# sanweiliti/EgoHMR

Hardware: AMD Instinct MI355X
Metric: sampled bodies/sec (100-step DDPM, batch 256) (higher is better)
Workload: dtype f32 results: denoiser GEMMs as 3x f16 MFMA on hi/lo-split operands (f32 accumulate) on the last 100 of 100 steps, plain f16 operands on the first 0; k = 100 is~; 1 GPU; B256 S1 DDPM-100 N4096 ResNet50+PointNet cond, diffuse_fuse(2 GCN passes), LBS every step, unguided; items_per_gpu=256, samples_per_item=1, denoising_steps=100, scene_points=4096, lbs_every_step=True, collision_guided=False, gcn_precision=f16x3, f16x3_last_steps=100, parallelism=items sharded x1, one RCCL all-gather of [B,226] at the end

## Files before the change

### egohmr_amd/csrc/gcn.hip

```cpp
#include <stdlib.h>

#include "common.h"
#include "egohmr_hip.h"
#include "gcn_dev.h"
#include "internal.h"

namespace {

__global__ void pack_w_kernel(const float* __restrict__ W, float* __restrict__ Wp, int K, int N) {
  __shared__ float tile[32][33];
  int u = blockIdx.z;
  int k0 = blockIdx.y * 32, n0 = blockIdx.x * 32;
  int tx = threadIdx.x & 31, ty = threadIdx.x >> 5;
  for (int r = ty; r < 32; r += 8) {
    int k = k0 + r, n = n0 + tx;
    tile[r][tx] = (k < K && n < N) ? W[((size_t)u * K + k) * N + n] : 0.f;
  }
  __syncthreads();
  for (int r = ty; r < 32; r += 8) {
    int n = n0 + r, k = k0 + tx;
    if (n < N && k < K) {
      int nt = n >> 6, c = n & 63;
      Wp[((size_t)nt * 128 + u * 64 + c) * K + k] = tile[tx][r];
    }
// ... 139 lines not shown
#pragma unroll
      for (int u = 0; u < 2; ++u) b[u] = *(const f32x4*)(Bs + (rB + 64 * u) * BK + cB);
#pragma unroll
      for (int s = 0; s < 4; ++s) {
#pragma unroll
        for (int t = 0; t < 3; ++t) {
          acc0[t] = __builtin_amdgcn_mfma_f32_32x32x2f32(a[t][s], b[0][s], acc0[t], 0, 0, 0);
          acc1[t] = __builtin_amdgcn_mfma_f32_32x32x2f32(a[t][s], b[1][s], acc1[t], 0, 0, 0);
        }
      }
    }
  }

  const int n = n_tile * BNH + 32 * wn + mi;
  const size_t rowb = m0 + 96 * wm + 48 * h;
  float res0[kJ], res1[kJ];
#pragma unroll
  for (int j = 0; j < kJ; ++j) res0[j] = RES ? Res[(rowb + j) * (size_t)N + n] : 0.f;
  {
    float dj[kJ], mj[kJ];
    const float sh = L.shift[n];
#pragma unroll
    for (int j = 0; j < kJ; ++j) { dj[j] = L.D[j * N + n]; mj[j] = L.M1[j * N + n]; }
    __builtin_amdgcn_sched_barrier(0);
#pragma unroll
    for (int j = 0; j < kJ; ++j) {
#pragma unroll
      for (int beta = 0; beta < 2; ++beta) {
        const int q = 24 * beta + j;
        acc0[q >> 4][q & 15] = fmaf(dj[j], acc0[q >> 4][q & 15], sh);
        acc1[q >> 4][q & 15] *= mj[j];
      }
    }
  }
  __builtin_amdgcn_sched_barrier(0);
#pragma unroll
  for (int j = 0; j < kJ; ++j) res1[j] = RES ? Res[(rowb + 24 + j) * (size_t)N + n] : 0.f;
  __builtin_amdgcn_sched_barrier(0);
  {
    float d0[kJ], g1[kJ];
#pragma unroll
    for (int j = 0; j < kJ; ++j) { d0[j] = acc0[j >> 4][j & 15]; g1[j] = acc1[j >> 4][j & 15]; }
    gcn_mix_store<false>(d0, g1, res0, n, N, rowb, L.Aoff, Y, L.relu != 0);
  }
  __builtin_amdgcn_sched_barrier(0);
  {
    float d0[kJ], g1[kJ];
#pragma unroll
    for (int j = 0; j < kJ; ++j) { d0[j] = acc0[(24 + j) >> 4][(24 + j) & 15]; g1[j] = acc1[(24 + j) >> 4][(24 + j) & 15]; }
    gcn_mix_store<false>(d0, g1, res1, n, N, rowb + 24, L.Aoff, Y, L.relu != 0);
  }
}

template <int OUT>
__global__ __launch_bounds__(256) void gcn_input_kernel(GcnInputArgs a) {
  __shared__ __attribute__((aligned(16))) float T[kJ * 256];
  gcn_input_body<OUT>(T, blockIdx.x, blockIdx.y, a);
}

template <int OUT>
__global__ __launch_bounds__(256) void gcn_input_rows_kernel(GcnInputArgs a) {
  __shared__ __attribute__((aligned(16))) float T[kJ * 256];
  gcn_input_body<OUT, false, true>(T, (int)threadIdx.x, blockIdx.x, blockIdx.y, a, nullptr);
}


template <bool HALF_IN>
__global__ __launch_bounds__(256) void gcn_out_dot_kernel(const float* __restrict__ X, OutDev O, float* __restrict__ hs, int64_t rows) {
  __shared__ float part[4][16][16];
  gcn_out_dot_rows16<HALF_IN, 0>(X, O, hs, (int64_t)blockIdx.x * OUT_ROWS_PER_BLOCK, rows, part, (int)threadIdx.x);
}

__global__ __launch_bounds__(192) void gcn_out_mix_kernel(const float* __restrict__ hs, OutDev O, const uint8_t* __restrict__ vis,
                                                          float* __restrict__ x0, int B, int passes, const int32_t* __restrict__ mask_slot) {
  __shared__ float sh[2][kJ][12];
  __shared__ float outs[2][kJ][6];
  const int b = blockIdx.x, tid = threadIdx.x;
  const int slot = mask_slot ? mask_slot[b] : b;
  for (int i = tid; i < passes * kJ * 12; i += 192) {
    const int p = i / (kJ * 12), rem = i % (kJ * 12);
    sh[p][rem / 12][rem % 12] = (p == 1 && slot < 0) ? 0.f : hs[((size_t)(p ? B + slot : b) * kJ) * 12 + rem];
  }
  __syncthreads();
  for (int e = tid; e < passes * kJ * 6; e += 192) {
    const int p = e / (kJ * 6), j = (e / 6) % kJ, c = e % 6;
    const float s = O.A[j * kJ + j] * (O.M[j * 6 + c] * sh[p][j][c]);
    float t = 0.f;
    for (int jp = 0; jp < kJ; ++jp)
      if (jp != j) t = fmaf(O.A[j * kJ + jp], O.M[jp * 6 + c] * sh[p][jp][6 + c], t);
    outs[p][j][c] = s + t + O.bias[c];
  }
  __syncthreads();
  if (tid < kPoseDim) {
    const int j = tid / 6, c = tid % 6;
    float v = outs[0][j][c];
    if (passes == 2 && !vis[(size_t)b * kJ + j]) v = outs[1][j][c];
    x0[(size_t)b * kPoseDim + tid] = v;
  }
}

}

__global__ void pack_aoff_half_kernel(const float* __restrict__ Aoff, half8* __restrict__ out) {
  const int lane = threadIdx.x, i = lane & 31;
#pragma unroll
  for (int s = 0; s < 3; ++s) {
    half8 v;
#pragma unroll
    for (int c = 0; c < 8; ++c) {
      const int kk = 16 * s + 8 * (lane >> 5) + c;
// ... 102 lines not shown
    hipLaunchKernelGGL(pack_out_kernel, dim3((unsigned)ceil_div(12 * hid_dim, 256)), dim3(256), 0, st, adj, *output_conv,
                       g->out.Wt, g->out.M, g->out.A, g->out.bias);
    if (hipGetLastError() != hipSuccess) rc = EHM_EIO;
  }
  if (rc == 0 && num_hidden > 0) {
    if (hipMalloc(&g->hidden_dev, sizeof(LayerDev) * num_hidden) != hipSuccess ||
        hipMemcpyAsync(g->hidden_dev, g->hidden, sizeof(LayerDev) * num_hidden, hipMemcpyHostToDevice, st) != hipSuccess)
      rc = EHM_ENOMEM;
  }
  if (rc == 0 && (hipMalloc(&g->chain_sticky, 64) != hipSuccess || hipMemsetAsync(g->chain_sticky, 0, 64, st) != hipSuccess)) rc = EHM_ENOMEM;
  if (rc == 0 && hipStreamSynchronize(st) != hipSuccess) rc = EHM_EIO;
  if (rc == 0) rc = ehm_gcn_reserve_rows(g, 2 * 256 * kJ);
  if (rc != 0) {
    if (g->hidden_dev) (void)hipFree(g->hidden_dev);
    if (g->chain_sticky) (void)hipFree(g->chain_sticky);
    if (g->chain_sync) (void)hipFree(g->chain_sync);
    if (g->hs) (void)hipFree(g->hs);
    (void)hipFree(g->arena);
    delete g;
    ehm_set_error("ehm_gcn_create: packing kernels failed");
    return rc;
  }
  *out = g;
  return 0;
}

extern "C" void ehm_gcn_destroy(ehm_gcn* h) {
  if (!h) return;
  (void)hipFree(h->arena);
  if (h->hs) (void)hipFree(h->hs);
  if (h->hidden_dev) (void)hipFree(h->hidden_dev);
  if (h->chain_sync) (void)hipFree(h->chain_sync);
  if (h->chain_sticky) (void)hipFree(h->chain_sticky);
  delete h;
}

int ehm_gcn_input_args(const ehm_gcn* h, const GcnRun& r, const float* h_img, const float* h_oth, const uint8_t* vis, const float* x, const float* Wx,
                       const float* tvec, float* out, int B, int passes, GcnInputArgs* a) {
  EHM_CHECK_ARG(h && h_img && h_oth && vis && x && Wx && tvec && out && a);
  EHM_CHECK_ARG(B > 0 && (passes == 1 || passes == 2));
  a->h_img = h_img; a->h_oth = h_oth; a->vis = vis; a->x = x; a->Wx = Wx; a->tvec = tvec;
  a->L = h->input;
  a->Y = out;
  a->B = B; a->passes = passes; a->mask_all = r.uncond_masks_all;
  a->mask_items = r.items(passes);
  a->sticky = h->chain_sticky;
  a->total_vb = r.virtual_bodies(B, passes);
  a->ny = (int)ceil_div(h->hid, 256);
  return 0;
}

template <bool PRE, int OUT>
static void launch_input_conv(const GcnInputArgs& a, hipStream_t st) {
  const dim3 grid((unsigned)a.total_vb, (unsigned)a.ny);
  if constexpr (PRE) hipLaunchKernelGGL(gcn_input_rows_kernel<OUT>, grid, dim3(256), 0, st, a);
  else hipLaunchKernelGGL(gcn_input_kernel<OUT>, grid, dim3(256), 0, st, a);
}
template <bool PRE>
static int input_conv(const GcnInputArgs& a, int fmt, hipStream_t st) {
  if (fmt == EHM_PREC_F32) launch_input_conv<PRE, 0>(a, st);
  else if (fmt == EHM_PREC_F16X3) launch_input_conv<PRE, 1>(a, st);
  else launch_input_conv<PRE, 2>(a, st);
  EHM_LAUNCH_CHECK();
  return 0;
}

int ehm_gcn_input_impl(const ehm_gcn* h, const GcnRun& r, const float* h_img, const float* h_oth, const uint8_t* vis, const float* x,
                       const float* Wx, const float* tvec, float* out, int B, int passes, hipStream_t st) {
  GcnInputArgs a;
  const int rc = ehm_gcn_input_args(h, r, h_img, h_oth, vis, x, Wx, tvec, out, B, passes, &a);
  return rc != 0 ? rc : input_conv<false>(a, gcn_input_format(h, r.precision), st);
}

extern "C" int ehm_gcn_input_layer(ehm_gcn* h, const float* h_img, const float* h_oth, const uint8_t* vis, const float* x,
                                   const float* Wx, const float* tvec, float* out, int B, int passes, void* stream) {
  EHM_CHECK_ARG(h);
  const int rc = ehm_gcn_input_impl(h, h->run, h_img, h_oth, vis, x, Wx, tvec, out, B, passes, (hipStream_t)stream);
  if (rc == 0) h->run.valid_rows = (int64_t)h->run.virtual_bodies(B, passes) * kJ;
  return rc;
}

extern "C" int ehm_gcn_input_layer_rows(ehm_gcn* h, const float* pre, float* out, int bodies, void* stream) {
  EHM_CHECK_ARG(h && pre && out && bodies > 0);
  GcnInputArgs a{};
  a.L = h->input;
  a.Y = out;
  a.B = bodies; a.passes = 1; a.mask_all = 0;
  a.mask_items = nullptr;
  a.total_vb = bodies;
  a.ny = (int)ceil_div(h->hid, 256);
  a.sticky = h->chain_sticky;
  h->run.valid_rows = (int64_t)bodies * kJ;
  a.pre = pre;
  return input_conv<true>(a, gcn_input_format(h, h->run.precision), (hipStream_t)stream);
}

static int hidden_layer(const ehm_gcn* h, const GcnRun& r, int layer, const float* X, const float* residual, float* out, int64_t rows_pad,
                        hipStream_t st) {
  EHM_CHECK_ARG(X && out);
  EHM_CHECK_ARG(layer >= 0 && layer < h->num_hidden);
  EHM_CHECK_ARG(rows_pad > 0 && rows_pad % BM == 0);
  EHM_CHECK_ARG(X != out);
  if (r.precision != EHM_PREC_F32)
    return ehm_gcn_tile_layer_impl(h, r, layer, X, residual, out, rows_pad, layer == h->num_hidden - 1, st);
  const int m_tiles = (int)(rows_pad / BM);
  const int blocks = m_tiles * (h->hid / BNH);
  if (residual)
    hipLaunchKernelGGL(gcn_hidden_kernel<true>, dim3(blocks), dim3(256), 0, st, X, h->hidden[layer], residual, out, m_tiles);
  else
    hipLaunchKernelGGL(gcn_hidden_kernel<false>, dim3(blocks), dim3(256), 0, st, X, h->hidden[layer], (const float*)nullptr, out, m_tiles);
  EHM_LAUNCH_CHECK();
  return 0;
}

extern "C" int ehm_gcn_hidden_layer(ehm_gcn* h, int layer, const float* X, const float* residual, float* out,
                                    int64_t rows_pad, void* stream) {
  EHM_CHECK_ARG(h);
  return hidden_layer(h, h->run, layer, X, residual, out, rows_pad, (hipStream_t)stream);
// ... 136 lines not shown
```

### egohmr_amd/csrc/gcn_dev.h

```cpp
#pragma once
#include "common.h"
#include "egohmr_hip.h"

typedef _Float16 half_t;
typedef _Float16 half8 __attribute__((ext_vector_type(8)));

constexpr int BM = 192;
constexpr int BNH = 64;
constexpr int BK = 32;
constexpr int A_TILE = BM * BK;
constexpr int B_TILE = 2 * BNH * BK;
constexpr int STAGE = A_TILE + B_TILE;

struct LayerDev {
  float* Wp;
  half_t* Ws;
  half_t* Wh;
  float* Ds;
  float* M1s;
  float w_scale;
  float* D;
  float* M1;
  float* shift;
  float* Aoff;
// ... 118 lines not shown
static __device__ __forceinline__ void gcn_mix_store(const float (&d0)[kJ], const float (&g1)[kJ], const float (&res)[kJ], int n, int N,
                                              size_t row0, const float* __restrict__ Aoff, float* __restrict__ Y, bool relu) {
  typedef const float __attribute__((address_space(4))) cfloat;
  const cfloat* Ac = (const cfloat*)(uintptr_t)Aoff;
#pragma unroll
  for (int j = 0; j < kJ; ++j) {
    float s = d0[j];
#pragma unroll
    for (int jp = 0; jp < kJ; ++jp) s = fmaf(Ac[j * kJ + jp], g1[jp], s);
    if (relu) s = fmaxf(s, 0.f);
    if (SPLIT_OUT) split_store_pair<G>((half_t*)Y, row0 + j, n, N, s + res[j]);
    else Y[(row0 + j) * (size_t)N + n] = s + res[j];
  }
}

typedef float f32x2 __attribute__((ext_vector_type(2)));
template <class Store>
static __device__ __forceinline__ void gcn_mix2(const f32x2 (&dp)[kJ], const f32x2 (&gp)[kJ], const float* __restrict__ Aoff, bool relu,
                                                Store store) {
  typedef const float __attribute__((address_space(4))) cfloat;
  const cfloat* Ac = (const cfloat*)(uintptr_t)Aoff;
#pragma unroll
  for (int j0 = 0; j0 < kJ; j0 += 4) {
    __builtin_amdgcn_sched_barrier(0);
#pragma unroll
    for (int i = 0; i < 4; ++i) {
      const int j = j0 + i;
      float s0 = dp[j][0], s1 = dp[j][1];
#pragma unroll
      for (int jp = 0; jp < kJ; ++jp) {
        const float a = Ac[j * kJ + jp];
        s0 = fmaf(a, gp[jp][0], s0);
        s1 = fmaf(a, gp[jp][1], s1);
      }
      if (relu) { s0 = fmaxf(s0, 0.f); s1 = fmaxf(s1, 0.f); }
      store(j, s0, s1);
    }
  }
}

constexpr unsigned int kStickySaturated = 4u;

struct GcnInputArgs {
  const float* h_img; const float* h_oth; const uint8_t* vis; const float* x; const float* Wx; const float* tvec;
  LayerDev L;
  float* Y;
  int B, passes, mask_all;
  const int32_t* mask_items;
  int total_vb, ny;
  unsigned int* sticky = nullptr;
  const float* pre = nullptr;
};

template <int OUT, bool X_LDS = false, bool PRE = false>
__device__ __forceinline__ void gcn_input_body(float* T, int tid, int bx, int by, const GcnInputArgs& a, const float* xb_in) {
  const float* __restrict__ h_img = a.h_img; const float* __restrict__ h_oth = a.h_oth; const uint8_t* __restrict__ vis = a.vis;
  const float* __restrict__ x = a.x; const float* __restrict__ Wx = a.Wx; const float* __restrict__ tvec = a.tvec;
  const LayerDev& L = a.L;
  float* __restrict__ Y = a.Y;
  const int B = a.B, passes = a.passes, mask_all = a.mask_all;
  const int32_t* __restrict__ mask_items = a.mask_items;
  (void)passes;
  const int N = L.N;
  const int vb = bx;
  const int p = vb >= B ? 1 : 0, b = p ? (mask_items ? mask_items[vb - B] : vb - B) : vb;
  const int n_raw = by * 256 + tid;
  const int n = n_raw < N ? n_raw : N - 1;
  float base[2] = {0.f, 0.f}, img[2] = {0.f, 0.f}, wx[2][6] = {{0.f, 0.f, 0.f, 0.f, 0.f, 0.f}, {0.f, 0.f, 0.f, 0.f, 0.f, 0.f}};
  if constexpr (!PRE)
#pragma unroll
  for (int k = 0; k < 2; ++k) {
    base[k] = ((p == 1 && mask_all) ? 0.f : h_oth[((size_t)b * 2 + k) * N + n]) + tvec[k * N + n];
    img[k] = (p == 0) ? h_img[((size_t)b * 2 + k) * N + n] : 0.f;
#pragma unroll
    for (int c = 0; c < 6; ++c) wx[k][c] = Wx[(k * 6 + c) * N + n];
  }
  const float* xb = xb_in ? xb_in : (PRE ? nullptr : x + (size_t)b * kPoseDim);
  float xr[X_LDS ? kPoseDim : 1];
  if constexpr (X_LDS) {
    typedef const f32x4 __attribute__((address_space(3))) lf32x4;
    lf32x4* xl = (lf32x4*)xb_in;
#pragma unroll
    for (int i = 0; i < kPoseDim / 4; ++i) {
      const f32x4 v = xl[i];
      xr[4 * i] = v[0]; xr[4 * i + 1] = v[1]; xr[4 * i + 2] = v[2]; xr[4 * i + 3] = v[3];
    }
  }
  const uint8_t* vb_ = PRE ? nullptr : vis + (size_t)b * kJ;
  float h0[kJ], h1[kJ];
  const float sh = L.shift[n];
  float dj[kJ], mj[kJ];
  {
    typedef unsigned int u32x4_tb __attribute__((ext_vector_type(4)));
    const __amdgpu_buffer_rsrc_t dsB = ehm_buffer_rsrc(L.Ds), m1B = ehm_buffer_rsrc(L.M1s);
    const unsigned int nrow = (unsigned int)n * (unsigned int)(kJ * 4);
#pragma unroll
    for (int q4 = 0; q4 < kJ / 4; ++q4) {
      const u32x4_tb d4 = __builtin_amdgcn_raw_buffer_load_b128(dsB, nrow, 16 * q4, 0);
      const u32x4_tb m4 = __builtin_amdgcn_raw_buffer_load_b128(m1B, nrow, 16 * q4, 0);
#pragma unroll
      for (int i = 0; i < 4; ++i) {
        const unsigned int du = d4[i], mu = m4[i];
        dj[4 * q4 + i] = __builtin_bit_cast(float, du);
        mj[4 * q4 + i] = __builtin_bit_cast(float, mu);
      }
    }
  }
  const f32x2 img2 = {img[0], img[1]}, base2 = {base[0], base[1]};
  f32x2 wx2[6];
#pragma unroll
  for (int c = 0; c < 6; ++c) wx2[c] = f32x2{wx[0][c], wx[1][c]};
#pragma unroll
  for (int j = 0; j < kJ; ++j) {
    f32x2 s;
    if constexpr (PRE) {
      const float* pr = a.pre + ((size_t)vb * kJ + j) * 2 * (size_t)N + n;
      s = f32x2{pr[0], pr[N]};
    } else {
    const float v = vb_[j] ? 1.f : 0.f;
    s = __builtin_elementwise_fma(f32x2{v, v}, img2, base2);
#pragma unroll
    for (int c = 0; c < 6; ++c) {
      const float xv = X_LDS ? xr[X_LDS ? j * 6 + c : 0] : xb[j * 6 + c];
      s = __builtin_elementwise_fma(f32x2{xv, xv}, wx2[c], s);
    }
    }
    h0[j] = fmaf(dj[j], s[0], sh);
    h1[j] = mj[j] * s[1];
  }
  if constexpr (OUT == 2) {
    typedef unsigned int u32x4_t __attribute__((ext_vector_type(4)));
    typedef _Float16 half2_t __attribute__((ext_vector_type(2)));
    const int lane = tid & 63, wv = tid >> 6;
    f32x16 DA, DB;
#pragma unroll
    for (int r = 0; r < 16; ++r) { DA[r] = 0.f; DB[r] = 0.f; }
#pragma unroll
    for (int s3 = 0; s3 < 3; ++s3) {
      const half8 af = ((const half8*)L.AoffH)[s3 * 64 + lane];
      u32x4_t Pw, Qw;
#pragma unroll
      for (int e = 0; e < 4; ++e) {
        const int kp = 16 * s3 + 2 * e, kq = kp + 8;
        const float p0 = kp < kJ ? h1[kp] : h0[kp - kJ], p1 = kp + 1 < kJ ? h1[kp + 1] : h0[kp + 1 - kJ];
        const float q0 = kq < kJ ? h1[kq] : h0[kq - kJ], q1 = kq + 1 < kJ ? h1[kq + 1] : h0[kq + 1 - kJ];
        const half2_t hp = {(half_t)fmaf(p0, 0.f, fminf(fmaxf(p0, -65504.f), 65504.f)), (half_t)fmaf(p1, 0.f, fminf(fmaxf(p1, -65504.f), 65504.f))};
        const half2_t hq = {(half_t)fmaf(q0, 0.f, fminf(fmaxf(q0, -65504.f), 65504.f)), (half_t)fmaf(q1, 0.f, fminf(fmaxf(q1, -65504.f), 65504.f))};
        const auto sw = __builtin_amdgcn_permlane32_swap(__builtin_bit_cast(unsigned int, hp), __builtin_bit_cast(unsigned int, hq), false, false);
        Pw[e] = sw[0];
        Qw[e] = sw[1];
      }
      DA = __builtin_amdgcn_mfma_f32_32x32x16_f16(af, __builtin_bit_cast(half8, Pw), DA, 0, 0, 0);
      DB = __builtin_amdgcn_mfma_f32_32x32x16_f16(af, __builtin_bit_cast(half8, Qw), DB, 0, 0, 0);
    }
    const bool relu = L.relu != 0;
    const int cA = 64 * wv + (lane & 31), half = lane >> 5;
#pragma unroll
    for (int r = 0; r < 12; ++r) {
      const int j = (r & 3) + 8 * (r >> 2) + 4 * half;
      const float va = relu ? fmaxf(DA[r], 0.f) : DA[r], vb = relu ? fmaxf(DB[r], 0.f) : DB[r];
      T[j * 256 + cA] = fmaf(DA[r], 0.f, va);
      T[j * 256 + cA + 32] = fmaf(DB[r], 0.f, vb);
    }
  } else {
    typedef const float __attribute__((address_space(4))) cfloat;
    const cfloat* Ac = (const cfloat*)(uintptr_t)L.Aoff;
    const bool relu = L.relu != 0;
    f32x2 sacc[kJ / 2];
#pragma unroll
    for (int jj = 0; jj < kJ / 2; ++jj) sacc[jj] = f32x2{h0[2 * jj], h0[2 * jj + 1]};
#pragma unroll
    for (int jp = 0; jp < kJ; ++jp) {
      const f32x2 hh = {h1[jp], h1[jp]};
#pragma unroll
      for (int jj = 0; jj < kJ / 2; ++jj) sacc[jj] = __builtin_elementwise_fma(f32x2{Ac[jp * kJ + 2 * jj], Ac[jp * kJ + 2 * jj + 1]}, hh, sacc[jj]);
    }
#pragma unroll
    for (int jj = 0; jj < kJ / 2; ++jj) {
      f32x2 o = sacc[jj];
      if (relu) { o[0] = fmaxf(o[0], 0.f); o[1] = fmaxf(o[1], 0.f); }
      if constexpr (OUT != 0) o = __builtin_elementwise_fma(sacc[jj], f32x2{0.f, 0.f}, o);
      T[(2 * jj) * 256 + tid] = o[0];
      T[(2 * jj + 1) * 256 + tid] = o[1];
    }
  }
  __syncthreads();
  typedef unsigned int u32x4 __attribute__((ext_vector_type(4)));
  const int nb = by * 256;
#pragma unroll
  for (int i = 0; i < 3; ++i) {
    const int u = tid + 256 * i, j = u >> 5, c8 = (u & 31) * 8;
    if (nb + c8 >= N) continue;

    const f32x4 v0 = *(const f32x4*)(T + j * 256 + c8), v1 = *(const f32x4*)(T + j * 256 + c8 + 4);
    const float v[8] = {v0[0], v0[1], v0[2], v0[3], v1[0], v1[1], v1[2], v1[3]};
    const size_t row = (size_t)vb * kJ + j;
    if (OUT != 0) {
      if (a.sticky) {
        float vm = 0.f;
#pragma unroll
        for (int k = 0; k < 8; k += 2) vm = fmaxf(vm, fmaxf(fabsf(v[k]), fabsf(v[k + 1])));
        if (vm >= 65504.f && vm <= 3.0e38f) __hip_atomic_fetch_or(a.sticky, kStickySaturated, __ATOMIC_RELAXED, __HIP_MEMORY_SCOPE_AGENT);
      }
      half8 hh, ll;
#pragma unroll
      for (int k = 0; k < 8; ++k) {
        const float c = fmaf(v[k], 0.f, fminf(fmaxf(v[k], -65504.f), 65504.f));
        hh[k] = (half_t)c;
        ll[k] = (half_t)fminf(fmaxf(v[k] - (float)hh[k], -65504.f), 65504.f);
      }
      if (OUT == 1) {
        half_t* p = (half_t*)Y + split_off<32>(row, nb + c8, N);
        *(u32x4*)p = __builtin_bit_cast(u32x4, hh);
        *(u32x4*)(p + 32) = __builtin_bit_cast(u32x4, ll);
      } else {
        *(u32x4*)((half_t*)Y + row * (size_t)N + nb + c8) = __builtin_bit_cast(u32x4, hh);
      }
    } else {
      float* p = Y + row * (size_t)N + nb + c8;
      *(f32x4*)p = v0;
      *(f32x4*)(p + 4) = v1;
    }
  }
}
template <int OUT>
__device__ __forceinline__ void gcn_input_body(float* T, int bx, int by, const GcnInputArgs& a) {
  gcn_input_body<OUT>(T, (int)threadIdx.x, bx, by, a, nullptr);
}

constexpr int OUT_ROWS_PER_BLOCK = 16;
template <bool HALF_IN, int AUX>
__device__ __forceinline__ f32x4 gcn_out_dot_quarter(const float* __restrict__ X, const OutDev& O, int64_t r, int wave, int lane) {
  const int K = O.K;
  const int row = lane & 15, q = lane >> 4;
  const int kq = K / 4;
  typedef unsigned int u32x4_od __attribute__((ext_vector_type(4)));
  typedef unsigned int u32x2_od __attribute__((ext_vector_type(2)));
  const __amdgpu_buffer_rsrc_t rsX = ehm_buffer_rsrc_4g(X), rsW = ehm_buffer_rsrc(O.Wt);
  const unsigned int vox = (unsigned int)((r * K + (size_t)wave * kq + 8 * q) * (HALF_IN ? 2 : 4));
  const unsigned int vow = (unsigned int)(((size_t)(row < 12 ? row : 0) * K + (size_t)wave * kq + 8 * q) * 4);
  f32x4 acc = {0.f, 0.f, 0.f, 0.f}, acc2 = {0.f, 0.f, 0.f, 0.f};
#pragma unroll 4
  for (int k = 0; k + 32 <= kq; k += 32) {
    float xv[8];
    if (HALF_IN) {
      const half8 hv = __builtin_bit_cast(half8, (u32x4_od)__builtin_amdgcn_raw_buffer_load_b128(rsX, vox, k * 2, AUX));
#pragma unroll
      for (int c = 0; c < 8; ++c) xv[c] = (float)hv[c];
    } else {
      const f32x4 x0 = __builtin_bit_cast(f32x4, (u32x4_od)__builtin_amdgcn_raw_buffer_load_b128(rsX, vox, k * 4, AUX));
      const f32x4 x1 = __builtin_bit_cast(f32x4, (u32x4_od)__builtin_amdgcn_raw_buffer_load_b128(rsX, vox, k * 4 + 16, AUX));
#pragma unroll
      for (int c = 0; c < 4; ++c) { xv[c] = x0[c]; xv[4 + c] = x1[c]; }
    }
    f32x4 w0 = __builtin_bit_cast(f32x4, (u32x4_od)__builtin_amdgcn_raw_buffer_load_b128(rsW, vow, k * 4, 0));
    f32x4 w1 = __builtin_bit_cast(f32x4, (u32x4_od)__builtin_amdgcn_raw_buffer_load_b128(rsW, vow, k * 4 + 16, 0));
    if (row >= 12) { w0 = f32x4{0.f, 0.f, 0.f, 0.f}; w1 = w0; }
#pragma unroll
    for (int c = 0; c < 4; c += 2) {
      acc = __builtin_amdgcn_mfma_f32_16x16x4f32(xv[c], w0[c], acc, 0, 0, 0);
      acc2 = __builtin_amdgcn_mfma_f32_16x16x4f32(xv[c + 1], w0[c + 1], acc2, 0, 0, 0);
    }
#pragma unroll
    for (int c = 0; c < 4; c += 2) {
      acc = __builtin_amdgcn_mfma_f32_16x16x4f32(xv[4 + c], w1[c], acc, 0, 0, 0);
      acc2 = __builtin_amdgcn_mfma_f32_16x16x4f32(xv[5 + c], w1[c + 1], acc2, 0, 0, 0);
    }
  }
  if (kq & 16) {
    const int k = kq - 16 - 4 * q;
    f32x4 xv;
    if (HALF_IN) {
      typedef _Float16 half4_t __attribute__((ext_vector_type(4)));
      const half4_t hv = __builtin_bit_cast(half4_t, (u32x2_od)__builtin_amdgcn_raw_buffer_load_b64(rsX, vox + (unsigned int)(k * 2), 0, AUX));
      xv = f32x4{(float)hv[0], (float)hv[1], (float)hv[2], (float)hv[3]};
    } else {
// ... 31 lines not shown
```

### egohmr_amd/csrc/internal.h

```cpp
#pragma once
#include "common.h"
#include "egohmr_hip.h"

int ehm_smpl_forward_impl(ehm_smpl* h, const float* betas, const float* rot_or_x, bool from_rot6d, const float* mean,
                          const float* std_, float* verts, float* joints, float* Rws, float* Aws, float* pose6d_out, int B,
                          hipStream_t st, float* vposed = nullptr);
int ehm_smpl_writes_vposed(const ehm_smpl* h, int B);
int ehm_smpl_pose_impl(ehm_smpl* h, const float* betas, const float* x, const float* mean, const float* std_, float* Rws, float* Aws,
                       float* jws, int B, hipStream_t st);
int ehm_step_body_impl(ehm_smpl* h, const float* hs, const void* out_dev, const uint8_t* vis, const float* x, const float* noise,
                       const float* grad, float* x_next, float* x0, const ehm_step_coefs* c, int ddim, int passes, const int32_t* mask_slot, int do_pose,
                       const float* betas, const float* mean, const float* std_, float* verts, float* joints, float* Rws, float* Aws,
                       float* pose6d, int B, hipStream_t st, const struct GcnInputArgs* next_input = nullptr, int next_prec = 0,
                       int* fused = nullptr, void* defer_pf = nullptr);
int ehm_skin_steps_impl(ehm_smpl* h, const float* A_steps, const void* pf_steps, int nsteps, int final_step, int B, float* verts, float* joints,
                        float* scratch_verts, float* scratch_joints, hipStream_t st);
int ehm_step_fused_impl(const void* out_dev, const float* X, int prec, const uint8_t* vis, const float* x, const float* noise, const float* grad,
                        float* x_next, float* x0, const ehm_step_coefs* c, int ddim, int passes, const int32_t* mask_slot, int B,
                        const struct GcnInputArgs* next_input, int next_prec, hipStream_t st);
int ehm_pose_steps_impl(ehm_smpl* smpl, const float* x0_steps, int nsteps, int final_step, int B, const float* betas, const float* mean,
                        const float* std_, float* A_steps, void* pf_steps, float* R, float* joints, float* pose6d, float* x0_final,
                        float* scratch_joints, hipStream_t st);
int ehm_skin_min_bodies();
int ehm_smpl_has_mfma_skin(const ehm_smpl* h);
int64_t ehm_skin_pf_bytes_per_step(int B);
void ehm_smpl_dev(const ehm_smpl* h, void* out);
size_t ehm_smpl_dev_size();
int ehm_smpl_num_verts(const ehm_smpl* h);
int ehm_smpl_num_extra(const ehm_smpl* h);
struct GcnInputArgs;
struct GcnRun;
int ehm_gcn_input_args(const ehm_gcn* h, const GcnRun& r, const float* h_img, const float* h_oth, const uint8_t* vis, const float* x, const float* Wx,
                       const float* tvec, float* out, int B, int passes, GcnInputArgs* a);
int ehm_gcn_input_impl(const ehm_gcn* h, const GcnRun& r, const float* h_img, const float* h_oth, const uint8_t* vis, const float* x,
                       const float* Wx, const float* tvec, float* out, int B, int passes, hipStream_t st);
int ehm_gcn_hidden_stack_impl(ehm_gcn* h, const GcnRun& r, float* const bufs[3], int64_t rows_pad, int* result_index, hipStream_t st);
int ehm_gcn_output_dot_impl(ehm_gcn* h, const GcnRun& r, const float* X, int B, int passes, const float** hs, hipStream_t st);
int ehm_num_cus();
int ehm_gcn_tile_layer_impl(const ehm_gcn* h, const GcnRun& r, int layer, const void* X, const void* residual, void* out, int64_t rows_pad,
                            bool out_f32, hipStream_t st);
int ehm_gcn_tile_chain_impl(ehm_gcn* h, const GcnRun& r, void* const bufs[3], int64_t rows_pad, hipStream_t st);
void ehm_pack_half(const float* X, void* Y, size_t n, float scale, hipStream_t st);
int ehm_gcn_reserve_rows(ehm_gcn* h, int64_t rows_pad);
int64_t ehm_guidance_scratch_bytes(int B, int N);
int ehm_guidance_impl(ehm_smpl* smpl, const float* betas, const float* x, const float* mean, const float* std_,
                      const float* scene, int B, int N, float tau, float denom, float margin, float* verts_ws, float* joints_ws, float* R_ws,
                      float* A_ws, float* gverts, float* loss, float* gpose, float* grad, void* scratch, hipStream_t st,
                      float* vposed_ws = nullptr);
unsigned long long* ehm_prof_evals_ptr();
struct EhmProfScope {
  int cls;
  hipStream_t st;
  void* rec;
  EhmProfScope(int cls_, hipStream_t st_);
  ~EhmProfScope();
};
```

### egohmr_amd/csrc/step.hip

```cpp
#include "common.h"
#include "egohmr_hip.h"
#include "gcn_dev.h"
#include "internal.h"
#include "smpl_dev.h"
#include "step_dev.h"

namespace {

struct StepFusedArgs {
  const float* X;
  StepBodyArgs sb;
  GcnInputArgs in;
  int do_input;
};

constexpr int kFusedT = kJ * 256;

template <bool HALF_IN, int OUT, int NT>
__global__ __launch_bounds__(NT, 4) void step_fused_kernel(StepFusedArgs a) {
  constexpr int G = NT / 256, NWV = NT / 64;
  __shared__ __attribute__((aligned(16))) float T[G * kFusedT];
  __shared__ __attribute__((aligned(16))) StepBodyLds L;
  const int tid = threadIdx.x, lane = tid & 63, wave = tid >> 6;
  const int b = blockIdx.x, B = a.sb.B;
  const int slot = a.sb.passes == 2 ? (a.sb.mask_slot ? a.sb.mask_slot[b] : b) : -1;
  const int nrows = slot >= 0 ? 2 * kJ : kJ;

  float (*part)[4][16][16] = (float (*)[4][16][16])T;
  for (int task = wave; task < 12; task += NWV) {
    const int tile = task >> 2, wq = task & 3;
    if (16 * tile < nrows) {
      int rr = 16 * tile + (lane & 15);
      if (rr >= nrows) rr = nrows - 1;
      const int64_t r = (int64_t)(rr >= kJ ? B + slot : b) * kJ + (rr % kJ);
      const f32x4 acc = gcn_out_dot_quarter<HALF_IN, 0>(a.X, a.sb.O, r, wq, lane);
#pragma unroll
      for (int c = 0; c < 4; ++c) part[tile][wq][4 * (lane >> 4) + c][lane & 15] = acc[c];
    }
  }
  if (wave == NWV - 1) step_stage_tables<true>(b, lane, a.sb, L);
  __syncthreads();
  for (int i = tid; i < 2 * kJ * 12; i += NT) {
    const int rr = i / 12, cc12 = i % 12, tile = rr >> 4, tr = rr & 15;
    (&L.sh[0][0][0])[i] = rr < nrows ? (part[tile][0][tr][cc12] + part[tile][1][tr][cc12]) + (part[tile][2][tr][cc12] + part[tile][3][tr][cc12]) : 0.f;
  }
  __syncthreads();
  if (wave < 3) {
    SmplDev unused;
    step_body_one<true, false, true>(b, lane, a.sb, unused, L, [] {}, wave, 3);
  }
  if (!a.do_input) return;
  __syncthreads();
  const int ny = a.in.ny, np = slot >= 0 ? 2 : 1, grp = tid >> 8;
  const int rounds = np * ((ny + G - 1) / G);
  for (int k = 0; k < rounds; ++k) {
    const int cb = grp + G * (k / np), p = k % np;
    if (cb < ny) gcn_input_body<OUT, true>(T + grp * kFusedT, tid & 255, p ? B + slot : b, cb, a.in, L.xn);
    else __syncthreads();
    __syncthreads();
  }
}

struct PoseStepsArgs {
  const float* x0_steps;
  const float *betas, *mean, *std_;
  float* A_steps; char* pf_steps; int64_t pf_bytes;
  float *R, *joints, *pose6d, *x0_final, *scratch_joints;
  int B, final_step, jstride;
};

__global__ __launch_bounds__(64) void pose_steps_kernel(PoseStepsArgs p, SmplDev S) {
  __shared__ StepBodyLds L;
  const int b = blockIdx.x, s = blockIdx.y, lane = threadIdx.x;
  const bool fin = s == p.final_step;
  StepBodyArgs a{};
  a.betas = p.betas; a.mean = p.mean; a.std_ = p.std_; a.B = p.B; a.jstride = p.jstride;
  a.Rws = fin ? p.R : nullptr;
  a.joints = fin ? p.joints : p.scratch_joints;
  a.pose6d = fin ? p.pose6d : nullptr;
  a.Aws = p.A_steps + (size_t)s * p.B * kJ * 12;
  a.pf = (sk_half8*)(p.pf_steps + (size_t)s * p.pf_bytes);
  const float* x0row = p.x0_steps + ((size_t)s * p.B + b) * kPoseDim;
  for (int e = lane; e < kPoseDim; e += 64) {
    const float v = x0row[e];
    L.x0s[e] = v;
    if (fin) p.x0_final[(size_t)b * kPoseDim + e] = v;
  }
  __syncthreads();
  step_pose_part(b, lane, a, S, L, [] { __syncthreads(); }, L.x0s);
}

template <bool HALF_IN, int NT>
void launch_fused2(int next_prec, int B, hipStream_t st, const StepFusedArgs& a) {
  const dim3 grid((unsigned)B), blk(NT);
  if (next_prec == EHM_PREC_F32) hipLaunchKernelGGL((step_fused_kernel<HALF_IN, 0, NT>), grid, blk, 0, st, a);
  else if (next_prec == EHM_PREC_F16X3) hipLaunchKernelGGL((step_fused_kernel<HALF_IN, 1, NT>), grid, blk, 0, st, a);
  else hipLaunchKernelGGL((step_fused_kernel<HALF_IN, 2, NT>), grid, blk, 0, st, a);
}
template <bool HALF_IN>
void launch_fused(int next_prec, int B, hipStream_t st, const StepFusedArgs& a) {
  if (B <= ehm_num_cus()) launch_fused2<HALF_IN, 1024>(next_prec, B, st, a);
  else if (B > 2 * ehm_num_cus()) launch_fused2<HALF_IN, 256>(next_prec, B, st, a);
  else launch_fused2<HALF_IN, 512>(next_prec, B, st, a);
}

}

int ehm_step_fused_impl(const void* out_dev, const float* X, int prec, const uint8_t* vis, const float* x, const float* noise, const float* grad,
                        float* x_next, float* x0, const ehm_step_coefs* c, int ddim, int passes, const int32_t* mask_slot, int B,
                        const GcnInputArgs* next_input, int next_prec, hipStream_t st) {
  StepFusedArgs a{};
  a.X = X;
  a.sb.hs = nullptr; a.sb.O = *(const OutDev*)out_dev; a.sb.vis = vis; a.sb.x = x; a.sb.noise = noise; a.sb.grad = grad; a.sb.x_next = x_next;
  a.sb.x0 = x0; a.sb.c = *c; a.sb.ddim = ddim; a.sb.passes = passes; a.sb.B = B; a.sb.do_pose = 0; a.sb.mask_slot = mask_slot;
  a.sb.trace = nullptr; a.sb.pf = nullptr;
  if (a.sb.O.K % 64 != 0) {
    ehm_set_error("ehm_step_fused_impl: hidden width %d is not a multiple of 64", a.sb.O.K);
    return EHM_EINVAL;
  }
  a.do_input = next_input ? 1 : 0;
  if (next_input) a.in = *next_input;
  EhmProfScope ps(EHM_PROF_STEP_FUSED, st);
  if (prec == EHM_PREC_F16) launch_fused<true>(next_prec, B, st, a);
  else launch_fused<false>(next_prec, B, st, a);
  EHM_LAUNCH_CHECK();
  return 0;
}

int ehm_pose_steps_impl(ehm_smpl* smpl, const float* x0_steps, int nsteps, int final_step, int B, const float* betas, const float* mean,
                        const float* std_, float* A_steps, void* pf_steps, float* R, float* joints, float* pose6d, float* x0_final,
                        float* scratch_joints, hipStream_t st) {
  SmplDev sd;
  ehm_smpl_dev(smpl, &sd);
  PoseStepsArgs p{x0_steps, betas, mean, std_, A_steps, (char*)pf_steps, ehm_skin_pf_bytes_per_step(B), R, joints, pose6d, x0_final, scratch_joints,
                  B, final_step, (kJ + ehm_smpl_num_extra(smpl)) * 3};
  EhmProfScope ps(EHM_PROF_STEP_BODY, st);
  hipLaunchKernelGGL(pose_steps_kernel, dim3(B, nsteps), dim3(64), 0, st, p, sd);
  EHM_LAUNCH_CHECK();
  return 0;
}
```

Before: 2265 bodies/s.

## Split next-step GCN input conv out of fused step into persistent prefetching kernel

The next step's GCN input layer is removed from the fused per-body step kernel, which now only does the output reduction and pose tail with smaller LDS. The input layer becomes a separate persistent kernel sized to about two blocks per CU. Each block loops over virtual bodies with double-buffered LDS, prefetching the next body's pose, visibility and conditioning features while computing the current one, and per-channel constants are hoisted out of the loop. This aims to improve occupancy and hide global load latency, at the cost of an extra kernel launch per step and losing the fusion with the step kernel.

```diff
diff --git a/egohmr_amd/csrc/gcn.hip b/egohmr_amd/csrc/gcn.hip
--- a/egohmr_amd/csrc/gcn.hip
+++ b/egohmr_amd/csrc/gcn.hip
@@ -215,10 +215,63 @@
   }
 }
 
+constexpr int kInputBlocksPerCU = 2;
+constexpr int kInputStage = kPoseDim + kJ + 4;
 template <int OUT>
-__global__ __launch_bounds__(256) void gcn_input_kernel(GcnInputArgs a) {
+__global__ __launch_bounds__(256, kInputBlocksPerCU) void gcn_input_kernel(GcnInputArgs a) {
   __shared__ __attribute__((aligned(16))) float T[kJ * 256];
-  gcn_input_body<OUT>(T, blockIdx.x, blockIdx.y, a);
+  __shared__ __attribute__((aligned(16))) float xs[2][kInputStage];
+  __shared__ __attribute__((aligned(16))) f32x4 cs[2][256];
+  const int tid = threadIdx.x, by = blockIdx.y, G = (int)gridDim.x;
+  constexpr int kItemSlot = kPoseDim + kJ;
+  InputChan c;
+  gcn_input_chan(c, tid, by, a);
+  struct Raw { unsigned int x, v, i; };
+  auto fetch = [&](int vb, int b) -> Raw {
+    const int e = tid < kPoseDim ? tid : kPoseDim - 1;
+    Raw r;
+    r.x = __builtin_bit_cast(unsigned int, a.x[(size_t)b * kPoseDim + e]);
+    r.v = (unsigned int)a.vis[(size_t)b * kJ + e / 6];
+    r.i = (unsigned int)(vb + G < a.total_vb ? gcn_input_item(vb + G, a) : 0);
+    return r;
+  };
+  auto put = [&](float* dst, const Raw& r) {
+    if (tid < kPoseDim) {
+      dst[tid] = __builtin_bit_cast(float, r.x);
+      if (tid % 6 == 0) dst[kPoseDim + tid / 6] = __builtin_bit_cast(float, r.v);
+      if (tid == 0) dst[kItemSlot] = __builtin_bit_cast(float, r.i);
+    }
+  };
+  auto put_cond = [&](f32x4* dst, const float (&r)[4]) { dst[tid] = f32x4{r[0], r[1], r[2], r[3]}; };
+  int vb = blockIdx.x;
+  {
+    const int b = gcn_input_item(vb, a);
+    float r[4];
+    gcn_input_cond_raw(r, tid, vb, b, by, a);
+    put(xs[0], fetch(vb, b));
+    put_cond(cs[0], r);
+  }
+  __syncthreads();
+  for (int k = 0; vb < a.total_vb; ++k) {
+    const int cur = k & 1, nxt = cur ^ 1, nvb = vb + G;
+    const bool more = nvb < a.total_vb;
+    const int pvb = more ? nvb : 0, pb = more ? __builtin_bit_cast(int, xs[cur][kItemSlot]) : 0;
+    float rn[4];
+    gcn_input_cond_raw(rn, tid, pvb, pb, by, a);
+    const Raw xn = fetch(pvb, pb);
+    InputBody o;
+    {
+      const f32x4 r4 = cs[cur][tid];
+      const float r[4] = {r4[0], r4[1], r4[2], r4[3]};
+      gcn_input_cond_finish(o, r, c);
+    }
+    gcn_input_unit<OUT, true>(T, tid, vb, by, a, xs[cur], c, o, [&] {
+      put(xs[nxt], xn);
+      put_cond(cs[nxt], rn);
+    });
+    __syncthreads();
+    vb = nvb;
+  }
 }
 
 template <int OUT>
@@ -427,9 +480,13 @@
 
 template <bool PRE, int OUT>
 static void launch_input_conv(const GcnInputArgs& a, hipStream_t st) {
-  const dim3 grid((unsigned)a.total_vb, (unsigned)a.ny);
-  if constexpr (PRE) hipLaunchKernelGGL(gcn_input_rows_kernel<OUT>, grid, dim3(256), 0, st, a);
-  else hipLaunchKernelGGL(gcn_input_kernel<OUT>, grid, dim3(256), 0, st, a);
+  if constexpr (PRE) {
+    hipLaunchKernelGGL(gcn_input_rows_kernel<OUT>, dim3((unsigned)a.total_vb, (unsigned)a.ny), dim3(256), 0, st, a);
+  } else {
+    const int per_by = (int)ceil_div(kInputBlocksPerCU * ehm_num_cus(), a.ny);
+    const int nbx = a.total_vb < per_by ? a.total_vb : per_by;
+    hipLaunchKernelGGL(gcn_input_kernel<OUT>, dim3((unsigned)nbx, (unsigned)a.ny), dim3(256), 0, st, a);
+  }
 }
 template <bool PRE>
 static int input_conv(const GcnInputArgs& a, int fmt, hipStream_t st) {
@@ -439,6 +496,7 @@
   EHM_LAUNCH_CHECK();
   return 0;
 }
+int ehm_gcn_input_launch(const GcnInputArgs& a, int fmt, hipStream_t st) { return input_conv<false>(a, fmt, st); }
 
 int ehm_gcn_input_impl(const ehm_gcn* h, const GcnRun& r, const float* h_img, const float* h_oth, const uint8_t* vis, const float* x,
                        const float* Wx, const float* tvec, float* out, int B, int passes, hipStream_t st) {
diff --git a/egohmr_amd/csrc/gcn_dev.h b/egohmr_amd/csrc/gcn_dev.h
--- a/egohmr_amd/csrc/gcn_dev.h
+++ b/egohmr_amd/csrc/gcn_dev.h
@@ -194,44 +194,29 @@
   const float* pre = nullptr;
 };
 
-template <int OUT, bool X_LDS = false, bool PRE = false>
-__device__ __forceinline__ void gcn_input_body(float* T, int tid, int bx, int by, const GcnInputArgs& a, const float* xb_in) {
-  const float* __restrict__ h_img = a.h_img; const float* __restrict__ h_oth = a.h_oth; const uint8_t* __restrict__ vis = a.vis;
-  const float* __restrict__ x = a.x; const float* __restrict__ Wx = a.Wx; const float* __restrict__ tvec = a.tvec;
+struct InputChan {
+  float dj[kJ], mj[kJ];
+  float sh;
+  float tv[2];
+  f32x2 wx2[6];
+};
+template <bool PRE = false>
+__device__ __forceinline__ void gcn_input_chan(InputChan& c, int tid, int by, const GcnInputArgs& a) {
   const LayerDev& L = a.L;
-  float* __restrict__ Y = a.Y;
-  const int B = a.B, passes = a.passes, mask_all = a.mask_all;
-  const int32_t* __restrict__ mask_items = a.mask_items;
-  (void)passes;
   const int N = L.N;
-  const int vb = bx;
-  const int p = vb >= B ? 1 : 0, b = p ? (mask_items ? mask_items[vb - B] : vb - B) : vb;
   const int n_raw = by * 256 + tid;
   const int n = n_raw < N ? n_raw : N - 1;
-  float base[2] = {0.f, 0.f}, img[2] = {0.f, 0.f}, wx[2][6] = {{0.f, 0.f, 0.f, 0.f, 0.f, 0.f}, {0.f, 0.f, 0.f, 0.f, 0.f, 0.f}};
-  if constexpr (!PRE)
-#pragma unroll
-  for (int k = 0; k < 2; ++k) {
-    base[k] = ((p == 1 && mask_all) ? 0.f : h_oth[((size_t)b * 2 + k) * N + n]) + tvec[k * N + n];
-    img[k] = (p == 0) ? h_img[((size_t)b * 2 + k) * N + n] : 0.f;
-#pragma unroll
-    for (int c = 0; c < 6; ++c) wx[k][c] = Wx[(k * 6 + c) * N + n];
-  }
-  const float* xb = xb_in ? xb_in : (PRE ? nullptr : x + (size_t)b * kPoseDim);
-  float xr[X_LDS ? kPoseDim : 1];
-  if constexpr (X_LDS) {
-    typedef const f32x4 __attribute__((address_space(3))) lf32x4;
-    lf32x4* xl = (lf32x4*)xb_in;
-#pragma unroll
-    for (int i = 0; i < kPoseDim / 4; ++i) {
-      const f32x4 v = xl[i];
-      xr[4 * i] = v[0]; xr[4 * i + 1] = v[1]; xr[4 * i + 2] = v[2]; xr[4 * i + 3] = v[3];
-    }
-  }
-  const uint8_t* vb_ = PRE ? nullptr : vis + (size_t)b * kJ;
-  float h0[kJ], h1[kJ];
-  const float sh = L.shift[n];
-  float dj[kJ], mj[kJ];
+  c.sh = L.shift[n];
+  c.tv[0] = c.tv[1] = 0.f;
+#pragma unroll
+  for (int k = 0; k < 6; ++k) c.wx2[k] = f32x2{0.f, 0.f};
+  if constexpr (!PRE) {
+    const float* __restrict__ Wx = a.Wx; const float* __restrict__ tvec = a.tvec;
+#pragma unroll
+    for (int k = 0; k < 2; ++k) c.tv[k] = tvec[k * N + n];
+#pragma unroll
+    for (int k = 0; k < 6; ++k) c.wx2[k] = f32x2{Wx[k * N + n], Wx[(6 + k) * N + n]};
+  }
   {
     typedef unsigned int u32x4_tb __attribute__((ext_vector_type(4)));
     const __amdgpu_buffer_rsrc_t dsB = ehm_buffer_rsrc(L.Ds), m1B = ehm_buffer_rsrc(L.M1s);
@@ -243,15 +228,84 @@
 #pragma unroll
       for (int i = 0; i < 4; ++i) {
         const unsigned int du = d4[i], mu = m4[i];
-        dj[4 * q4 + i] = __builtin_bit_cast(float, du);
-        mj[4 * q4 + i] = __builtin_bit_cast(float, mu);
-      }
-    }
-  }
+        c.dj[4 * q4 + i] = __builtin_bit_cast(float, du);
+        c.mj[4 * q4 + i] = __builtin_bit_cast(float, mu);
+      }
+    }
+  }
+}
+
+__device__ __forceinline__ int gcn_input_item(int vb, const GcnInputArgs& a) {
+  return vb >= a.B ? (a.mask_items ? a.mask_items[vb - a.B] : vb - a.B) : vb;
+}
+struct InputBody {
+  float base[2], img[2];
+};
+__device__ __forceinline__ void gcn_input_cond_raw(float (&r)[4], int tid, int vb, int b , int by, const GcnInputArgs& a) {
+  const int N = a.L.N, p = vb >= a.B ? 1 : 0;
+  const int n_raw = by * 256 + tid;
+  const int n = n_raw < N ? n_raw : N - 1;
+#pragma unroll
+  for (int k = 0; k < 4; ++k) r[k] = 0.f;
+  if (!(p == 1 && a.mask_all)) {
+#pragma unroll
+    for (int k = 0; k < 2; ++k) r[k] = a.h_oth[((size_t)b * 2 + k) * N + n];
+  }
+  if (p == 0) {
+#pragma unroll
+    for (int k = 0; k < 2; ++k) r[2 + k] = a.h_img[((size_t)b * 2 + k) * N + n];
+  }
+}
+__device__ __forceinline__ void gcn_input_cond_finish(InputBody& o, const float (&r)[4], const InputChan& c) {
+#pragma unroll
+  for (int k = 0; k < 2; ++k) {
+    o.base[k] = r[k] + c.tv[k];
+    o.img[k] = r[2 + k];
+  }
+}
+
+struct InputNoMid { __device__ void operator()() const {} };
+template <int OUT, bool X_LDS = false, bool PRE = false, class Mid = InputNoMid>
+__device__ __forceinline__ void gcn_input_unit(float* T, int tid, int bx, int by, const GcnInputArgs& a, const float* xb_in, const InputChan& c,
+                                               const InputBody& o, Mid mid = Mid()) {
+  const uint8_t* __restrict__ vis = a.vis;
+  const float* __restrict__ x = a.x;
+  const LayerDev& L = a.L;
+  float* __restrict__ Y = a.Y;
+  const int N = L.N;
+  const int vb = bx;
+  const int b = gcn_input_item(vb, a);
+  const int n_raw = by * 256 + tid;
+  const int n = n_raw < N ? n_raw : N - 1;
+  const float (&base)[2] = o.base;
+  const float (&img)[2] = o.img;
+  const float* xb = xb_in ? xb_in : (PRE ? nullptr : x + (size_t)b * kPoseDim);
+  float xr[X_LDS ? kPoseDim : 1], vr[X_LDS ? kJ : 1];
+  if constexpr (X_LDS) {
+    typedef const f32x4 __attribute__((address_space(3))) lf32x4;
+    lf32x4* xl = (lf32x4*)xb_in;
+#pragma unroll
+    for (int i = 0; i < kPoseDim / 4; ++i) {
+      const f32x4 v = xl[i];
+      xr[4 * i] = v[0]; xr[4 * i + 1] = v[1]; xr[4 * i + 2] = v[2]; xr[4 * i + 3] = v[3];
+    }
+#pragma unroll
+    for (int i = 0; i < kJ / 4; ++i) {
+      const f32x4 v = xl[kPoseDim / 4 + i];
+#pragma unroll
+      for (int e = 0; e < 4; ++e) {
+        const float ve = v[e];
+        vr[4 * i + e] = __builtin_bit_cast(unsigned int, ve) ? 1.f : 0.f;
+      }
+    }
+  }
+  const uint8_t* vb_ = (PRE || X_LDS) ? nullptr : vis + (size_t)b * kJ;
+  float h0[kJ], h1[kJ];
+  const float sh = c.sh;
+  const float (&dj)[kJ] = c.dj;
+  const float (&mj)[kJ] = c.mj;
   const f32x2 img2 = {img[0], img[1]}, base2 = {base[0], base[1]};
-  f32x2 wx2[6];
-#pragma unroll
-  for (int c = 0; c < 6; ++c) wx2[c] = f32x2{wx[0][c], wx[1][c]};
+  const f32x2 (&wx2)[6] = c.wx2;
 #pragma unroll
   for (int j = 0; j < kJ; ++j) {
     f32x2 s;
@@ -259,7 +313,7 @@
       const float* pr = a.pre + ((size_t)vb * kJ + j) * 2 * (size_t)N + n;
       s = f32x2{pr[0], pr[N]};
     } else {
-    const float v = vb_[j] ? 1.f : 0.f;
+    const float v = X_LDS ? vr[X_LDS ? j : 0] : (vb_[j] ? 1.f : 0.f);
     s = __builtin_elementwise_fma(f32x2{v, v}, img2, base2);
 #pragma unroll
     for (int c = 0; c < 6; ++c) {
@@ -306,7 +360,9 @@
     }
   } else {
     typedef const float __attribute__((address_space(4))) cfloat;
-    const cfloat* Ac = (const cfloat*)(uintptr_t)L.Aoff;
+    uint64_t aoff = (uint64_t)(uintptr_t)L.Aoff;
+    asm volatile("" : "+s"(aoff));
+    const cfloat* Ac = (const cfloat*)(uintptr_t)aoff;
     const bool relu = L.relu != 0;
     f32x2 sacc[kJ / 2];
 #pragma unroll
@@ -326,6 +382,7 @@
       T[(2 * jj + 1) * 256 + tid] = o[1];
     }
   }
+  mid();
   __syncthreads();
   typedef unsigned int u32x4 __attribute__((ext_vector_type(4)));
   const int nb = by * 256;
@@ -364,6 +421,18 @@
       *(f32x4*)(p + 4) = v1;
     }
   }
+}
+template <int OUT, bool X_LDS = false, bool PRE = false>
+__device__ __forceinline__ void gcn_input_body(float* T, int tid, int bx, int by, const GcnInputArgs& a, const float* xb_in) {
+  InputChan c;
+  gcn_input_chan<PRE>(c, tid, by, a);
+  InputBody o{};
+  if constexpr (!PRE) {
+    float r[4];
+    gcn_input_cond_raw(r, tid, bx, gcn_input_item(bx, a), by, a);
+    gcn_input_cond_finish(o, r, c);
+  }
+  gcn_input_unit<OUT, X_LDS, PRE>(T, tid, bx, by, a, xb_in, c, o);
 }
 template <int OUT>
 __device__ __forceinline__ void gcn_input_body(float* T, int bx, int by, const GcnInputArgs& a) {
diff --git a/egohmr_amd/csrc/internal.h b/egohmr_amd/csrc/internal.h
--- a/egohmr_amd/csrc/internal.h
+++ b/egohmr_amd/csrc/internal.h
@@ -34,6 +34,7 @@
                        const float* tvec, float* out, int B, int passes, GcnInputArgs* a);
 int ehm_gcn_input_impl(const ehm_gcn* h, const GcnRun& r, const float* h_img, const float* h_oth, const uint8_t* vis, const float* x,
                        const float* Wx, const float* tvec, float* out, int B, int passes, hipStream_t st);
+int ehm_gcn_input_launch(const GcnInputArgs& a, int fmt, hipStream_t st);
 int ehm_gcn_hidden_stack_impl(ehm_gcn* h, const GcnRun& r, float* const bufs[3], int64_t rows_pad, int* result_index, hipStream_t st);
 int ehm_gcn_output_dot_impl(ehm_gcn* h, const GcnRun& r, const float* X, int B, int passes, const float** hs, hipStream_t st);
 int ehm_num_cus();
diff --git a/egohmr_amd/csrc/step.hip b/egohmr_amd/csrc/step.hip
--- a/egohmr_amd/csrc/step.hip
+++ b/egohmr_amd/csrc/step.hip
@@ -10,23 +10,18 @@
 struct StepFusedArgs {
   const float* X;
   StepBodyArgs sb;
-  GcnInputArgs in;
-  int do_input;
 };
 
-constexpr int kFusedT = kJ * 256;
-
-template <bool HALF_IN, int OUT, int NT>
+template <bool HALF_IN, int NT>
 __global__ __launch_bounds__(NT, 4) void step_fused_kernel(StepFusedArgs a) {
-  constexpr int G = NT / 256, NWV = NT / 64;
-  __shared__ __attribute__((aligned(16))) float T[G * kFusedT];
+  constexpr int NWV = NT / 64;
+  __shared__ __attribute__((aligned(16))) float part[3][4][16][16];
   __shared__ __attribute__((aligned(16))) StepBodyLds L;
   const int tid = threadIdx.x, lane = tid & 63, wave = tid >> 6;
   const int b = blockIdx.x, B = a.sb.B;
   const int slot = a.sb.passes == 2 ? (a.sb.mask_slot ? a.sb.mask_slot[b] : b) : -1;
   const int nrows = slot >= 0 ? 2 * kJ : kJ;
 
-  float (*part)[4][16][16] = (float (*)[4][16][16])T;
   for (int task = wave; task < 12; task += NWV) {
     const int tile = task >> 2, wq = task & 3;
     if (16 * tile < nrows) {
@@ -48,16 +43,6 @@
   if (wave < 3) {
     SmplDev unused;
     step_body_one<true, false, true>(b, lane, a.sb, unused, L, [] {}, wave, 3);
-  }
-  if (!a.do_input) return;
-  __syncthreads();
-  const int ny = a.in.ny, np = slot >= 0 ? 2 : 1, grp = tid >> 8;
-  const int rounds = np * ((ny + G - 1) / G);
-  for (int k = 0; k < rounds; ++k) {
-    const int cb = grp + G * (k / np), p = k % np;
-    if (cb < ny) gcn_input_body<OUT, true>(T + grp * kFusedT, tid & 255, p ? B + slot : b, cb, a.in, L.xn);
-    else __syncthreads();
-    __syncthreads();
   }
 }
 
@@ -90,18 +75,10 @@
   step_pose_part(b, lane, a, S, L, [] { __syncthreads(); }, L.x0s);
 }
 
-template <bool HALF_IN, int NT>
-void launch_fused2(int next_prec, int B, hipStream_t st, const StepFusedArgs& a) {
-  const dim3 grid((unsigned)B), blk(NT);
-  if (next_prec == EHM_PREC_F32) hipLaunchKernelGGL((step_fused_kernel<HALF_IN, 0, NT>), grid, blk, 0, st, a);
-  else if (next_prec == EHM_PREC_F16X3) hipLaunchKernelGGL((step_fused_kernel<HALF_IN, 1, NT>), grid, blk, 0, st, a);
-  else hipLaunchKernelGGL((step_fused_kernel<HALF_IN, 2, NT>), grid, blk, 0, st, a);
-}
 template <bool HALF_IN>
-void launch_fused(int next_prec, int B, hipStream_t st, const StepFusedArgs& a) {
-  if (B <= ehm_num_cus()) launch_fused2<HALF_IN, 1024>(next_prec, B, st, a);
-  else if (B > 2 * ehm_num_cus()) launch_fused2<HALF_IN, 256>(next_prec, B, st, a);
-  else launch_fused2<HALF_IN, 512>(next_prec, B, st, a);
+void launch_tail(int B, hipStream_t st, const StepFusedArgs& a) {
+  if (B <= ehm_num_cus()) hipLaunchKernelGGL((step_fused_kernel<HALF_IN, 1024>), dim3((unsigned)B), dim3(1024), 0, st, a);
+  else hipLaunchKernelGGL((step_fused_kernel<HALF_IN, 256>), dim3((unsigned)B), dim3(256), 0, st, a);
 }
 
 }
@@ -118,13 +95,11 @@
     ehm_set_error("ehm_step_fused_impl: hidden width %d is not a multiple of 64", a.sb.O.K);
     return EHM_EINVAL;
   }
-  a.do_input = next_input ? 1 : 0;
-  if (next_input) a.in = *next_input;
   EhmProfScope ps(EHM_PROF_STEP_FUSED, st);
-  if (prec == EHM_PREC_F16) launch_fused<true>(next_prec, B, st, a);
-  else launch_fused<false>(next_prec, B, st, a);
+  if (prec == EHM_PREC_F16) launch_tail<true>(B, st, a);
+  else launch_tail<false>(B, st, a);
   EHM_LAUNCH_CHECK();
-  return 0;
+  return next_input ? ehm_gcn_input_launch(*next_input, next_prec, st) : 0;
 }
 
 int ehm_pose_steps_impl(ehm_smpl* smpl, const float* x0_steps, int nsteps, int final_step, int B, const float* betas, const float* mean,
```

After: 2288 bodies/s, median of 6. No clear change (+1.0%).
